# LayerXcom/zero-chain

Measured on AMD Instinct MI355X. Metric: Groth16 proofs/sec (Transfer circuit), higher is better.
Workload: dtype u32 limbs (Fq 381-bit: 14 x 28-bit; Fr 255-bit: 8 x 32-bit; modular integer arithmetic)

## Files before the change

### zero-chain_amd/csrc/msm_asm_g1.h

```cpp
#pragma once
#include "msm_accumulate.h"
#ifdef ZK_HAVE_MADD_ASM
#include "madd_asm.h"
#include "red_asm.h"

namespace zkdev {

ZK_DI void g1asm_task(uint32_t t, const Affine<Fq28>* __restrict__ table, const uint32_t* __restrict__ pairs,
                       const uint4* __restrict__ sorted, XYZZ<Fq28>* __restrict__ tsums, uint32_t* __restrict__ n_redo,
                       uint32_t* __restrict__ redo) {
    static_assert(ZK_MADD_G1_VGPRS <= 168, "the loop must fit three waves per SIMD");
    static_assert(XYZZ<Fq28>::BX >= 9 && XYZZ<Fq28>::BY >= 5, "bounds of the values handed back by the loop");
    const uint4 d = sorted[t];
    const uint32_t n = d.z;
    XYZZ<Fq28> acc = XYZZ<Fq28>::inf();
    if (n) {
        const uint32_t* pp = pairs + d.x;
        const uint32_t pr = pp[0];
        const Affine<Fq28> p = table[pr >> 1];
        if (n == 1) {
            acc = XYZZ<Fq28>{p.x, (pr & 1u) ? neg_b<Fq28::MO>(p.y) : p.y, Fq28::one(), Fq28::one()};
        } else {
            u32x16 X = fq28_vec(p.x), Y = fq28_vec(p.y), ZZ = fq28_vec(Fq28::one()), ZZZ = ZZ;
            if (pr & 1u) {
// ... 2 lines not shown
            }
            const uint64_t pa = (uint64_t)(uintptr_t)pp, ta = (uint64_t)(uintptr_t)table;
            X[14] = (uint32_t)pa;
            X[15] = (uint32_t)(pa >> 32);
            Y[14] = n;
            ZZ[14] = (uint32_t)ta;
            ZZ[15] = (uint32_t)(ta >> 32);
            asm volatile(ZK_MADD_G1_ASM
                         : "+{v[0:15]}"(X), "+{v[16:31]}"(Y), "+{v[32:47]}"(ZZ), "+{v[48:63]}"(ZZZ)
                         :
                         : ZK_MADD_G1_ASM_CLOBBERS);
            acc.x = fq28_from_signed<7, false>(X);
            acc.y = ((n - 1) & 1u) ? fq28_from_signed<3, true>(Y)
                                   : fq28_from_signed<2, false>(Y);
            acc.zz = fq28_from_signed_product(ZZ);
            acc.zzz = fq28_from_signed_product(ZZZ);
            if (acc.zz.is_zero_norm()) redo[atomicAdd(n_redo, 1u)] = t;
        }
    }
    tsums[d.y] = acc;
}
static __global__ void __launch_bounds__(128, 3)
k_msm_accumulate_g1asm(const Affine<Fq28>* __restrict__ table, const uint32_t* __restrict__ pairs,
                       const uint4* __restrict__ sorted, const uint32_t* __restrict__ total, XYZZ<Fq28>* __restrict__ tsums,
                       uint32_t* __restrict__ n_redo, uint32_t* __restrict__ redo) {
    const uint32_t t = blockIdx.x * blockDim.x + threadIdx.x;
    if (t < total[0]) g1asm_task(t, table, pairs, sorted, tsums, n_redo, redo);
}
static __global__ void __launch_bounds__(128, 3)
k_msm_accumulate_g1asm_persistent(const Affine<Fq28>* __restrict__ table, const uint32_t* __restrict__ pairs,
                                  const uint4* __restrict__ sorted, const uint32_t* __restrict__ total,
                                  XYZZ<Fq28>* __restrict__ tsums, uint32_t* __restrict__ n_redo, uint32_t* __restrict__ redo,
                                  uint32_t* __restrict__ next) {
    const uint32_t ntask = total[0], lane = threadIdx.x & 63u;
    for (;;) {
        uint32_t base = 0;
        if (lane == 0) base = atomicAdd(next, 64u);
        base = __builtin_amdgcn_readfirstlane(base);
        if (base >= ntask) break;
        if (base + lane < ntask) g1asm_task(base + lane, table, pairs, sorted, tsums, n_redo, redo);
    }
}

ZK_DI XYZZ<Fq28> red_asm_point(const u32x16& x, const u32x16& y, const u32x16& zz, const u32x16& zzz, bool is_inf, bool raw) {
    if (is_inf) return XYZZ<Fq28>::inf();
    if (raw) return XYZZ<Fq28>{fq28_unvec(x), fq28_unvec(y), fq28_unvec(zz), fq28_unvec(zzz)};
    return XYZZ<Fq28>{fq28_from_signed<7, false>(x),
                      fq28_from_signed<2, false>(y),
                      fq28_from_signed_product(zz), fq28_from_signed_product(zzz)};
}
static __global__ void __launch_bounds__(64, 2)
k_msm_reduce1_g1asm(const XYZZ<Fq28>* __restrict__ tsums, const uint32_t* __restrict__ cnt, const uint32_t* __restrict__ toff,
                    const uint32_t* __restrict__ task_base, XYZZ<Fq28>* __restrict__ S, XYZZ<Fq28>* __restrict__ A, uint32_t nb,
                    uint32_t L, uint32_t* __restrict__ n_fallback) {
    static_assert(ZK_RED_G1_VGPRS <= 256, "the loop must fit two waves per SIMD");
    static_assert(sizeof(XYZZ<Fq28>) == 224, "the loop loads 224-byte partial sums");
    const uint32_t T = nb / L;
    const uint32_t bx = (blockIdx.x + blockIdx.y) % gridDim.x;
    const uint32_t t = bx * blockDim.x + threadIdx.x;
    if (t >= T) return;
    const uint32_t job = blockIdx.y;
    const size_t b0 = (size_t)job * nb + (size_t)t * L;
    const XYZZ<Fq28>* ts = tsums + task_base[job];
    u32x16 X = {}, Y = {}, ZZ = {}, ZZZ = {}, AX, AY, AZZ, AZZZ;
    const uint64_t pc = (uint64_t)(uintptr_t)(cnt + b0), pt = (uint64_t)(uintptr_t)(toff + b0), pp = (uint64_t)(uintptr_t)ts;
    X[14] = (uint32_t)pc;
    X[15] = (uint32_t)(pc >> 32);
    Y[14] = (uint32_t)pt;
    Y[15] = (uint32_t)(pt >> 32);
    ZZ[14] = (uint32_t)pp;
    ZZ[15] = (uint32_t)(pp >> 32);
    ZZZ[14] = L;
    asm volatile(ZK_RED_G1_ASM
                 : "+{v[0:15]}"(X), "+{v[16:31]}"(Y), "+{v[32:47]}"(ZZ), "+{v[48:63]}"(ZZZ), "={v[64:79]}"(AX), "={v[80:95]}"(AY),
                   "={v[96:111]}"(AZZ), "={v[112:127]}"(AZZZ)
                 :
                 : ZK_RED_G1_ASM_CLOBBERS);
    const uint32_t flags = ZZZ[15];
    XYZZ<Fq28> run = red_asm_point(X, Y, ZZ, ZZZ, (flags & ZK_RED_FLAG_RUN_INF) != 0, (flags & ZK_RED_FLAG_RUN_RAW) != 0);
    XYZZ<Fq28> acc = red_asm_point(AX, AY, AZZ, AZZZ, (flags & ZK_RED_FLAG_ACC_INF) != 0, (flags & ZK_RED_FLAG_ACC_RAW) != 0);
    if ((!(flags & ZK_RED_FLAG_RUN_INF) && run.zz.is_zero_norm()) || (!(flags & ZK_RED_FLAG_ACC_INF) && acc.zz.is_zero_norm())) {
        atomicAdd(n_fallback, 1u);
        run = XYZZ<Fq28>::inf();
        acc = XYZZ<Fq28>::inf();
        for (int k = (int)L - 1; k >= 0; k--) {
            if (cnt[b0 + k]) run = xadd(run, ts[toff[b0 + k]]);
            if (k >= 1) acc = xadd(acc, run);
        }
    }
    S[(size_t)job * T + t] = run;
    A[(size_t)job * T + t] = acc;
}
static __global__ void __launch_bounds__(64, 2)
k_msm_reduce1_g1asm_sf(const XYZZ<Fq28>* __restrict__ tsums, const uint32_t* __restrict__ cnt, const uint32_t* __restrict__ toff,
                       const uint32_t* __restrict__ task_base, XYZZ<Fq28>* __restrict__ S, XYZZ<Fq28>* __restrict__ A, uint32_t nb,
                       uint32_t L, uint32_t* __restrict__ n_fallback, uint32_t* __restrict__ fallback) {
    const uint32_t T = nb / L;
    const uint32_t bx = (blockIdx.x + blockIdx.y) % gridDim.x;
    const uint32_t t = bx * 64u + lane_of_wave(0u);
    if (t >= T) return;
    const uint32_t job = blockIdx.y;
    size_t b0 = (size_t)job * nb + (size_t)t * L;
    const XYZZ<Fq28>* ts = tsums + task_base[job];
    u32x16 X = {}, Y = {}, ZZ = {}, ZZZ = {}, AX, AY, AZZ, AZZZ;
    const uint64_t pc = (uint64_t)(uintptr_t)(cnt + b0), pt = (uint64_t)(uintptr_t)(toff + b0), pp = (uint64_t)(uintptr_t)ts;
    X[14] = (uint32_t)pc;
    X[15] = (uint32_t)(pc >> 32);
    Y[14] = (uint32_t)pt;
    Y[15] = (uint32_t)(pt >> 32);
    ZZ[14] = (uint32_t)pp;
    ZZ[15] = (uint32_t)(pp >> 32);
    ZZZ[14] = L;
    asm volatile(ZK_RED_G1_ASM
                 : "+{v[0:15]}"(X), "+{v[16:31]}"(Y), "+{v[32:47]}"(ZZ), "+{v[48:63]}"(ZZZ), "={v[64:79]}"(AX), "={v[80:95]}"(AY),
                   "={v[96:111]}"(AZZ), "={v[112:127]}"(AZZZ)
                 :
                 : ZK_RED_G1_ASM_CLOBBERS_MIN);
    uint32_t opaque0 = 0;
    asm volatile("" : "+s"(opaque0));
    const uint32_t t2 = bx * 64u + lane_of_wave(opaque0);
    const uint32_t flags = ZZZ[15];
    XYZZ<Fq28> run = red_asm_point(X, Y, ZZ, ZZZ, (flags & ZK_RED_FLAG_RUN_INF) != 0, (flags & ZK_RED_FLAG_RUN_RAW) != 0);
    XYZZ<Fq28> acc = red_asm_point(AX, AY, AZZ, AZZZ, (flags & ZK_RED_FLAG_ACC_INF) != 0, (flags & ZK_RED_FLAG_ACC_RAW) != 0);
    if ((!(flags & ZK_RED_FLAG_RUN_INF) && run.zz.is_zero_norm()) || (!(flags & ZK_RED_FLAG_ACC_INF) && acc.zz.is_zero_norm()))
        fallback[atomicAdd(n_fallback, 1u)] = job * T + t2;
    S[(size_t)job * T + t2] = run;
    A[(size_t)job * T + t2] = acc;
}
static __global__ void __launch_bounds__(64, MsmOcc<Fq28>::red)
k_msm_reduce1_redo(const XYZZ<Fq28>* __restrict__ tsums, const uint32_t* __restrict__ cnt, const uint32_t* __restrict__ toff,
                   const uint32_t* __restrict__ task_base, XYZZ<Fq28>* __restrict__ S, XYZZ<Fq28>* __restrict__ A, uint32_t nb,
                   uint32_t L, const uint32_t* __restrict__ n_fallback, const uint32_t* __restrict__ fallback) {
    const uint32_t T = nb / L, n = n_fallback[0];
    for (uint32_t i = blockIdx.x * blockDim.x + threadIdx.x; i < n; i += gridDim.x * blockDim.x) {
        const uint32_t node = fallback[i], job = node / T, t = node % T;
        const size_t b0 = (size_t)job * nb + (size_t)t * L;
        const XYZZ<Fq28>* ts = tsums + task_base[job];
        XYZZ<Fq28> run = XYZZ<Fq28>::inf(), acc = XYZZ<Fq28>::inf();
        for (int k = (int)L - 1; k >= 0; k--) {
            if (cnt[b0 + k]) run = xadd(run, ts[toff[b0 + k]]);
            if (k >= 1) acc = xadd(acc, run);
        }
        S[node] = run;
        A[node] = acc;
    }
}

}
#endif
```

### zero-chain_amd/csrc/msm_g1.cpp

```cpp
#define ZK_MSM_GROUP_INSTANTIATE 1
#include "msm_group_impl.h"
#include "msm_sort.h"
#include "msm_asm_g1.h"

namespace zkrt {

zk_status msm_sort_pairs(const MsmPlan& p, hipStream_t st, const MsmSortBufs& w, uint32_t nb, uint32_t c, const zkdev::MsmRecode& rc,
                         const zkdev::MsmSelSet& sel_set) {
    const size_t nj = p.nj;
    const MsmJob* dj = w.jobs;
    if (p.lds_sort) {
        ProfScope ps("msm_sort_lds", st);
        ZK_LAUNCH_SYNC(zkdev::k_msm_sort_lds, dim3((unsigned)nj), dim3(zkdev::MSM_SORT_THREADS), (size_t)nb * 4, st, dj, c, w.cnt, w.off, w.toff,
                       w.ntasks, w.pairs, p.seg, hook_env("ZKAMD_DEBUG_SORT") ? (uint32_t)atoi(hook_env("ZKAMD_DEBUG_SORT")) : 0u, sel_set, rc);
        return ZK_OK;
    }
    const uint32_t fine_log = p.fine_log, fine = 1u << fine_log, n_coarse = p.n_coarse, per_wg = zkdev::MSM_COARSE_SCALARS;
    const dim3 gridc(p.coarse_wgs, (unsigned)nj);
    uint32_t* coarse_cnt = w.coarse;
    uint32_t* coarse_off = coarse_cnt + nj * (size_t)n_coarse;
    uint32_t* bin_tasks = coarse_off + nj * (size_t)n_coarse;
    uint32_t* bin_tbase = bin_tasks + nj * (size_t)n_coarse;
    HIP_TRY(hipMemsetAsync(coarse_cnt, 0, nj * (size_t)n_coarse * 4, st));
    {
        ProfScope ps("msm_sort_coarse", st);
        ZK_LAUNCH_SYNC(zkdev::k_msm_coarse_count, gridc, dim3(256), 0, st, dj, c, fine_log, n_coarse, coarse_cnt, w.blockbase, per_wg, sel_set, rc);
        ZK_LAUNCH_SYNC(zkdev::k_msm_coarse_scan, dim3((unsigned)nj), dim3(zkdev::MSM_SORT_THREADS), 0, st,
                       (const uint32_t*)coarse_cnt, coarse_off, (uint32_t*)nullptr, n_coarse);
        ZK_LAUNCH_SYNC(zkdev::k_msm_coarse_scatter, gridc, dim3(256), 0, st, dj, c, fine_log, n_coarse,
                       (const uint32_t*)coarse_off, (const uint32_t*)w.blockbase, w.rank, per_wg, sel_set, rc);
    }
    {
        ProfScope ps("msm_sort_fine", st);
        ZK_LAUNCH_SYNC(zkdev::k_msm_fine_sort, dim3(n_coarse, (unsigned)nj), dim3(zkdev::MSM_SORT_THREADS), 0, st, dj,
                       (const uint2*)w.rank, (const uint32_t*)coarse_cnt, (const uint32_t*)coarse_off, fine, nb, w.cnt, w.off, w.toff,
                       bin_tasks, w.pairs, p.seg);
        ZK_LAUNCH_SYNC(zkdev::k_msm_coarse_scan, dim3((unsigned)nj), dim3(zkdev::MSM_SORT_THREADS), 0, st,
                       (const uint32_t*)bin_tasks, bin_tbase, w.ntasks, n_coarse);
        ZK_LAUNCH(zkdev::k_msm_task_offsets, dim3((nb + 255) / 256, (unsigned)nj), dim3(256), 0, st, w.toff,
                  (const uint32_t*)bin_tbase, nb, fine_log, n_coarse);
    }
    return ZK_OK;
}

zk_status msm_order_tasks(const MsmPlan& p, hipStream_t st, const MsmSortBufs& w, uint32_t nb) {
    const uint32_t nj = (uint32_t)p.nj;
    const dim3 gridb((nb + 255) / 256, nj);
    uint32_t* lenhist = w.hist;
    uint32_t* cursor = lenhist + p.n_class;
    ProfScope ps("msm_task_sort", st);
    ZK_LAUNCH_SYNC(zkdev::k_msm_task_hist, gridb, dim3(256), 0, st, w.cnt, lenhist, nb, p.seg);
    ZK_LAUNCH_SYNC(zkdev::k_msm_task_base, dim3(1), dim3(zkdev::MSM_SORT_THREADS), 0, st, lenhist, w.tclass, w.n_tasks, nj, p.seg);
    ZK_LAUNCH_SYNC(zkdev::k_msm_task_place, gridb, dim3(256), 0, st, w.cnt, w.off, w.toff, w.tbase, w.tclass, cursor, w.sorted, w.n_heavy,
                   w.heavy, nb, nj, p.merge_inline, p.seg, w.n_light, w.light);
    return ZK_OK;
}

#ifdef ZK_HAVE_RED_ASM
template <>
void launch_red_asm<zkdev::Fq28>(const zkdev::XYZZ<zkdev::Fq28>* tsums, const uint32_t* cnt, const uint32_t* toff, const uint32_t* tbase,
                                 zkdev::XYZZ<zkdev::Fq28>* S, zkdev::XYZZ<zkdev::Fq28>* A, uint32_t nb, uint32_t L, dim3 grid,
                                 hipStream_t st, uint32_t* n_fallback, uint32_t* fallback) {
    if (kernel_form(1)) {
        ZK_LAUNCH(zkdev::k_msm_reduce1_g1asm_sf, grid, dim3(64), 0, st, tsums, cnt, toff, tbase, S, A, nb, L, n_fallback, fallback);
        ZK_LAUNCH(zkdev::k_msm_reduce1_redo, dim3(256), dim3(64), 0, st, tsums, cnt, toff, tbase, S, A, nb, L, (const uint32_t*)n_fallback,
                  (const uint32_t*)fallback);
    } else {
        ZK_LAUNCH(zkdev::k_msm_reduce1_g1asm, grid, dim3(64), 0, st, tsums, cnt, toff, tbase, S, A, nb, L, n_fallback);
    }
}
#endif
#ifdef ZK_HAVE_MADD_ASM
int persist_wgs(int group) {
    static const int v1 = getenv("ZKAMD_G1_PERSIST") ? atoi(getenv("ZKAMD_G1_PERSIST")) : 6;
    static const int v2 = getenv("ZKAMD_G2_PERSIST") ? atoi(getenv("ZKAMD_G2_PERSIST")) : 4;
    return group == 2 ? v2 : v1;
}
template <>
void launch_asm_loop<zkdev::Fq28>(const zkdev::Affine<zkdev::Fq28>* table, const uint32_t* pairs, const uint4* sorted,
                                  const uint32_t* d_total, zkdev::XYZZ<zkdev::Fq28>* tsums, uint32_t* d_nredo, uint32_t* redo,
                                  unsigned blocks, hipStream_t st) {
    if (persist_wgs() > 0 && blocks > 256u * (unsigned)persist_wgs())
        ZK_LAUNCH(zkdev::k_msm_accumulate_g1asm_persistent, dim3(256u * (unsigned)persist_wgs()), dim3(128), 0, st, table, pairs, sorted,
                  d_total, tsums, d_nredo, redo, d_nredo + 1);
    else
        ZK_LAUNCH(zkdev::k_msm_accumulate_g1asm, dim3(blocks), dim3(128), 0, st, table, pairs, sorted, d_total, tsums, d_nredo, redo);
    ZK_LAUNCH_SYNC(zkdev::k_msm_accumulate_redo<zkdev::Fq28>, dim3(1024), dim3(64), 0, st, table, pairs, sorted,
                   (const uint32_t*)d_nredo, (const uint32_t*)redo, tsums);
}
#endif

zk_status calibrate_g1_reduce(const zkdev::Affine<zkdev::Fq28>* table, uint32_t n1, float ms[2]) {
#ifdef ZK_HAVE_RED_ASM
    typedef zkdev::XYZZ<zkdev::Fq28> P1;
    const uint32_t nj = 256, nb = 4096, L = 8, T = nb / L, n_sums = 1u << 16;
    DevBuf sums, cnt, toff, tbase, S, A, ctr, list;
    ZK_TRY(sums.ensure((size_t)n_sums * sizeof(P1)));
    ZK_TRY(cnt.ensure((size_t)nj * nb * 4));
    ZK_TRY(toff.ensure((size_t)nj * nb * 4));
    ZK_TRY(tbase.ensure(nj * 4));
    ZK_TRY(S.ensure((size_t)nj * T * sizeof(P1)));
    ZK_TRY(A.ensure((size_t)nj * T * sizeof(P1)));
    ZK_TRY(ctr.ensure(4));
    ZK_TRY(list.ensure((size_t)nj * T * 4));
    HIP_TRY(hipMemsetAsync(tbase.p, 0, nj * 4, g_stream));
    ZK_LAUNCH(zkdev::k_calib_buckets<zkdev::Fq28>, dim3(nj * nb / 256), dim3(256), 0, g_stream, table, n1, sums.as<P1>(), n_sums,
              cnt.as<uint32_t>(), toff.as<uint32_t>(), nj * nb);
    const dim3 grid(T / 64, nj);
    ZK_TRY(timed_best([&] {
        (void)hipMemsetAsync(ctr.p, 0, 4, g_stream);
        ZK_LAUNCH(zkdev::k_msm_reduce1_g1asm, grid, dim3(64), 0, g_stream, (const P1*)sums.as<P1>(), (const uint32_t*)cnt.as<uint32_t>(),
                  (const uint32_t*)toff.as<uint32_t>(), (const uint32_t*)tbase.as<uint32_t>(), S.as<P1>(), A.as<P1>(), nb, L, ctr.as<uint32_t>());
    }, &ms[0]));
    ZK_TRY(timed_best([&] {
        (void)hipMemsetAsync(ctr.p, 0, 4, g_stream);
        ZK_LAUNCH(zkdev::k_msm_reduce1_g1asm_sf, grid, dim3(64), 0, g_stream, (const P1*)sums.as<P1>(), (const uint32_t*)cnt.as<uint32_t>(),
                  (const uint32_t*)toff.as<uint32_t>(), (const uint32_t*)tbase.as<uint32_t>(), S.as<P1>(), A.as<P1>(), nb, L, ctr.as<uint32_t>(),
                  list.as<uint32_t>());
        ZK_LAUNCH(zkdev::k_msm_reduce1_redo, dim3(256), dim3(64), 0, g_stream, (const P1*)sums.as<P1>(), (const uint32_t*)cnt.as<uint32_t>(),
                  (const uint32_t*)toff.as<uint32_t>(), (const uint32_t*)tbase.as<uint32_t>(), S.as<P1>(), A.as<P1>(), nb, L,
                  (const uint32_t*)ctr.as<uint32_t>(), (const uint32_t*)list.as<uint32_t>());
    }, &ms[1]));
    HIP_TRY(hipStreamSynchronize(g_stream));
#else
    (void)table; (void)n1;
    ms[0] = ms[1] = 0.f;
#endif
    return ZK_OK;
}

ZK_MSM_GROUP_DEFINE(zkhost::Fq, zkdev::Fq)

}

#ifdef ZK_TEST_HOOKS
extern "C" zk_status zk_hook_msm_plan(int is_g2, uint32_t c, const uint32_t* n, size_t n_jobs, uint32_t vb_digit, int has_asm_loop,
                                      int has_asm_reduce, uint64_t* out, size_t out_words) try {
    using namespace zkrt;
    if (!n || !n_jobs || !out || c < 2 || c > 22) return fail(ZK_ERR_INVALID_ARGUMENT, "bad argument");
    std::vector<MsmJob> jobs(n_jobs, MsmJob{});
    for (size_t k = 0; k < n_jobs; k++) {
        jobs[k].n = n[k];
        jobs[k].vb_digit = vb_digit;
    }
    MsmPlan p;
    if (msm_plan(p, is_g2 != 0, c, 1u << (c - 2), vb_digit ? 1u : zkdev::msm_max_digits(c), jobs.data(), n_jobs, has_asm_loop != 0,
                 has_asm_reduce != 0, MsmTunables::read(is_g2 != 0)) != ZK_OK)
        return fail(p.status, p.refusal);
    const MsmPlan::Bytes& b = p.bytes;
    const uint64_t f[] = {p.seg, p.few, p.coop_l1, p.coop_rb, p.merge_inline, p.heavy_cap, p.light_cap, p.use_light, p.big_launch, p.acc_asm,
                          p.red_asm, p.L, p.T, p.nbits, p.log2_2l, p.s_stride, p.nsplit, p.lds_sort, p.fine_log, p.n_coarse, p.coarse_wgs,
                          p.heavy_blocks, p.medium_max, p.max_n, p.total, p.total_tasks, p.n_buckets, p.n_class,
                          b.jobs_d, b.bucket, b.per_job, b.hist, b.heavy, b.light, b.tclass, b.sorted, b.tsums, b.pairs, b.red_r, b.red_w, b.red_t,
                          b.pin_jobs, b.rank, b.blockbase, b.coarse, b.redo, b.result, n_jobs};
    const size_t nf = sizeof(f) / sizeof(f[0]);
    if (out_words < nf + 2 * n_jobs) return fail(ZK_ERR_INVALID_ARGUMENT, "output too short");
    std::copy(f, f + nf, out);
    std::copy(p.pair_base.begin(), p.pair_base.end(), out + nf);
    std::copy(p.tbase.begin(), p.tbase.end(), out + nf + n_jobs);
    return ZK_OK;
} ZK_ABI_CATCH
#endif
```

### zero-chain_amd/csrc/msm_group.h

```cpp
#pragma once
#include <stdio.h>
#include <stdlib.h>
#include <string.h>
#include <string>
#include <vector>
#include <algorithm>
#include <utility>
#include <mutex>
#include "../../include/zkamd.h"
#include "gpu_rt.h"
#include "host_common.h"
#include "host_math.h"
#include "msm_types.h"
#include "coop_tail.h"
#include "msm_plan.h"

namespace zkrt {

inline uint32_t pick_window(size_t n, int group) {
    const char* env = getenv(group == 2 ? "ZKAMD_WINDOW_BITS_G2" : group == 3 ? "ZKAMD_WINDOW_BITS_G1A" : "ZKAMD_WINDOW_BITS_G1");
    if (!env) env = getenv("ZKAMD_WINDOW_BITS");
    if (env && atoi(env) >= 2 && atoi(env) <= 22) return (uint32_t)atoi(env);
    const char* benv = getenv(group == 2 ? "ZKAMD_BUCKET_COST_G2" : "ZKAMD_BUCKET_COST_G1");
    const double beta = benv && atof(benv) > 0 ? atof(benv) : (group == 2 ? 12.0 : group == 1 ? 4.0 : 6.0);
    uint32_t best = 2;
    double best_cost = 1e300;
    for (uint32_t c = 2; c <= 22; c++) {
        double cost = 254.0 / (c + 1) * (double)(n ? n : 1) + beta * (double)((size_t)1 << (c - 2));
        if (cost < best_cost) {
            best_cost = cost;
            best = c;
        }
    }
    return best;
}

template <class HF, class DF>
zk_status check_points_dev(const zkdev::Affine<DF>* d_pts, size_t n, const char* what);
template <class HF, class DF>
zk_status check_points_host(const std::vector<zkhost::Affine<HF>>& pts, const char* what);
template <class DF>
zk_status import_affine_dev(const void* d_src, zkdev::Affine<DF>* dst, size_t n, hipStream_t st);
template <class DF>
zk_status build_table_dev(zkdev::Affine<DF>* table, size_t n, uint32_t npos, DevBuf& scratch, uint32_t n_mult, uint32_t j0, hipStream_t st);

struct KernelForms {
    bool done = false;
    uint32_t form[2] = {0, 0};
    float ms[4] = {0, 0, 0, 0};
};
inline std::mutex g_forms_mu;
inline KernelForms g_forms[64];
inline uint32_t kernel_form(int which) {
    static const int forced = [] {
        const char* e = getenv("ZKAMD_KERNEL_FORM");
        return !e ? -1 : !strcmp(e, "free") ? 1 : !strcmp(e, "scratch") ? 0 : -1;
    }();
    if (forced >= 0) return (uint32_t)forced;
    return g_forms[g_device & 63].form[which];
}

template <class DF>
constexpr bool asm_loop() { return false; }
template <class DF>
void launch_asm_loop(const zkdev::Affine<DF>*, const uint32_t*, const uint4*, const uint32_t*, zkdev::XYZZ<DF>*, uint32_t*,
                            uint32_t*, unsigned, hipStream_t) {}
template <class DF>
constexpr bool asm_reduce() { return false; }
template <class DF>
void launch_red_asm(const zkdev::XYZZ<DF>*, const uint32_t*, const uint32_t*, const uint32_t*, zkdev::XYZZ<DF>*, zkdev::XYZZ<DF>*,
                           uint32_t, uint32_t, dim3, hipStream_t, uint32_t*, uint32_t*) {}
#ifdef ZK_HAVE_RED_ASM
template <> constexpr bool asm_reduce<zkdev::Fq28>() { return true; }
template <>
void launch_red_asm<zkdev::Fq28>(const zkdev::XYZZ<zkdev::Fq28>* tsums, const uint32_t* cnt, const uint32_t* toff, const uint32_t* tbase,
                                 zkdev::XYZZ<zkdev::Fq28>* S, zkdev::XYZZ<zkdev::Fq28>* A, uint32_t nb, uint32_t L, dim3 grid,
                                 hipStream_t st, uint32_t* n_fallback, uint32_t* fallback);
#endif
#ifdef ZK_HAVE_MADD_ASM
int persist_wgs(int group = 1);
template <> constexpr bool asm_loop<zkdev::Fq28>() { return true; }
template <> constexpr bool asm_loop<zkdev::Fq2x>() { return true; }
template <>
void launch_asm_loop<zkdev::Fq28>(const zkdev::Affine<zkdev::Fq28>* table, const uint32_t* pairs, const uint4* sorted,
                                  const uint32_t* d_total, zkdev::XYZZ<zkdev::Fq28>* tsums, uint32_t* d_nredo, uint32_t* redo,
                                  unsigned blocks, hipStream_t st);
template <>
void launch_asm_loop<zkdev::Fq2x>(const zkdev::Affine<zkdev::Fq2x>* table, const uint32_t* pairs, const uint4* sorted,
                                  const uint32_t* d_total, zkdev::XYZZ<zkdev::Fq2x>* tsums, uint32_t* d_nredo, uint32_t* redo,
                                  unsigned blocks, hipStream_t st);
#endif

struct MsmSortBufs {
    const MsmJob* jobs;
    uint32_t *cnt, *off, *toff, *ntasks, *pairs, *blockbase, *coarse;
    uint2* rank;
    uint32_t *hist, *tclass, *tbase;
    uint4* sorted;
    uint32_t *heavy, *light;
    uint32_t *n_tasks, *n_heavy, *n_light;
};
zk_status msm_sort_pairs(const MsmPlan& p, hipStream_t st, const MsmSortBufs& w, uint32_t nb, uint32_t c, const zkdev::MsmRecode& rc,
                         const zkdev::MsmSelSet& sel_set);
zk_status msm_order_tasks(const MsmPlan& p, hipStream_t st, const MsmSortBufs& w, uint32_t nb);

template <class HF, class DF>
struct MsmGroup {
    typedef zkhost::Affine<HF> HAffine;
    typedef zkhost::Point<HF> HPoint;
    typedef zkdev::Affine<DF> DAffine;
// ... 133 lines not shown
```

### zero-chain_amd/csrc/msm_group_impl.h

```cpp
#pragma once
#include "msm_group.h"
#include "msm_accumulate.h"
#include "msm_reduce.h"
#include "msm_point_kernels.h"

namespace zkrt {

template <class DF>
zk_status import_affine_dev(const void* d_src, zkdev::Affine<DF>* dst, size_t n, hipStream_t st) {
    if (!n) return ZK_OK;
    ZK_LAUNCH(zkdev::k_import_affine<DF>, dim3((unsigned)((n + 127) / 128)), dim3(128), 0, st, (const uint32_t*)d_src, dst, (uint32_t)n);
    HIP_TRY(hipGetLastError());
    return ZK_OK;
}

template <class DF>
zk_status build_table_dev(zkdev::Affine<DF>* table, size_t n, uint32_t npos, DevBuf& scratch, uint32_t n_mult, uint32_t j0, hipStream_t st) {
    ZK_TRY(scratch.ensure((size_t)zkdev::MSM_TABLE_CHUNK * 5 * sizeof(DF) * n));
    ZK_LAUNCH(zkdev::k_msm_build_table<DF>, dim3((unsigned)((n + 127) / 128)), dim3(128), 0, st, table, (uint32_t)n, npos, scratch.as<DF>(),
              n_mult, j0);
    HIP_TRY(hipGetLastError());
    return ZK_OK;
}

// ... 267 lines not shown
    ZK_LAUNCH_SYNC(zkdev::k_msm_merge_heavy<DF>,
                   dim3(lane_heavy_blocks + (light_buckets + zkdev::MSM_MERGE_THREADS - 1) / zkdev::MSM_MERGE_THREADS),
                   dim3(zkdev::MSM_MERGE_THREADS), 0, st, (const uint32_t*)heavy.as<uint32_t>(), (const uint32_t*)d_nheavy,
                   (const uint32_t*)cnt.as<uint32_t>(), (const uint32_t*)toff.as<uint32_t>(),
                   (const uint32_t*)tbase.as<uint32_t>(), tsums.as<DPoint>(), nb, seg, lane_heavy_blocks, light_buckets,
                   merge_inline, min_heavy);
    if (p.use_light)
        ZK_LAUNCH_SYNC(zkdev::k_msm_merge_light<DF>, dim3((unsigned)std::min<size_t>((p.light_cap + 63) / 64, 2048)), dim3(64), 0, st,
                       (const uint32_t*)light.as<uint32_t>(), (const uint32_t*)counter(p, N_LIGHT), (const uint32_t*)cnt.as<uint32_t>(),
                       (const uint32_t*)toff.as<uint32_t>(), (const uint32_t*)tbase.as<uint32_t>(), tsums.as<DPoint>(), nb, seg);
    return ZK_OK;
}

template <class HF, class DF>
zk_status MsmGroup<HF, DF>::level1(const MsmPlan& p, hipStream_t st) {
    const uint32_t nj = (uint32_t)p.nj, L = p.L;
    const dim3 grid((p.T + 63) / 64, nj);
    DPoint *R = node_s(), *W = node_w();
    if (p.coop_l1) {
        zkcoop::level1<DF>(tsums.as<DPoint>(), cnt.as<uint32_t>(), toff.as<uint32_t>(), tbase.as<uint32_t>(), R, W, nb, L, nj, st);
    } else if (p.red_asm) {
        launch_red_asm<DF>(tsums.as<DPoint>(), cnt.as<uint32_t>(), toff.as<uint32_t>(), tbase.as<uint32_t>(), R, W, nb, L, grid, st,
                           counter(p, N_FALLBACK), redo.as<uint32_t>());
        if (hook_env("ZKAMD_DEBUG_REDO")) dump_redo(p, st, true);
    } else {
        ZK_LAUNCH(zkdev::k_msm_suffix_buckets<DF>, grid, dim3(64), 0, st, tsums.as<DPoint>(), cnt.as<uint32_t>(),
                  toff.as<uint32_t>(), tbase.as<uint32_t>(), R, nb, L, p.few ? 0u : 1u , p.seg);
        ZK_LAUNCH(zkdev::k_msm_segsum<DF>, grid, dim3(64), 0, st, (const DPoint*)R, (const DPoint*)nullptr, W, nb, L,
                  1u, 1u, 1u);
    }
    return ZK_OK;
}

template <class HF, class DF>
zk_status MsmGroup<HF, DF>::tail(const MsmPlan& p, hipStream_t st) {
    const uint32_t nj = (uint32_t)p.nj, nbits = p.nbits;
    if (p.few) {
        DPoint* parts = red_t.as<DPoint>();
        DPoint* Y = p.nsplit > 1 ? parts + p.nj * (size_t)(nbits + 1) * p.nsplit : parts;
        zkcoop::planes<DF>(node_s(), p.s_stride, node_w(), Y, parts, p.T, nbits, nj, st);
        zkcoop::combine<DF>(Y, job_sums(p), nbits, p.log2_2l, nj, st);
    } else {
        zkcoop::upper<DF>(node_s(), p.s_stride, node_w(), job_sums(p), p.T, p.log2_2l, p.red_asm, nj, st);
    }
    return ZK_OK;
}

template <class HF, class DF>
void MsmGroup<HF, DF>::dump_redo(const MsmPlan& p, hipStream_t st, bool after_level1) {
    (void)hipStreamSynchronize(st);
    if (after_level1) {
        uint32_t v[2] = {0, 0};
        (void)hipMemcpy(v, counter(p, N_LIGHT), 8, hipMemcpyDeviceToHost);
        fprintf(stderr, "[redo] reduction G1: %u buckets with 2..%u partials merged, %u of %zu level-1 nodes recomputed\n", v[0],
                p.merge_inline, v[1], p.nj * (size_t)p.T);
        return;
    }
    uint32_t nr = 0, tot = 0;
    (void)hipMemcpy(&nr, counter(p, N_REDO), 4, hipMemcpyDeviceToHost);
    (void)hipMemcpy(&tot, counter(p, N_TASKS), 4, hipMemcpyDeviceToHost);
    fprintf(stderr, "[redo] group %s: %u of %u tasks flagged\n", IS_G2 ? "G2" : "G1", nr, tot);
    for (uint32_t q = 0; q < nr && q < 6; q++) {
        uint32_t ti = 0;
        uint4 dsc;
        (void)hipMemcpy(&ti, redo.as<uint32_t>() + q, 4, hipMemcpyDeviceToHost);
        (void)hipMemcpy(&dsc, sorted.as<uint4>() + ti, 16, hipMemcpyDeviceToHost);
        std::vector<uint32_t> pw(dsc.z);
        (void)hipMemcpy(pw.data(), pairs.as<uint32_t>() + dsc.x, dsc.z * 4, hipMemcpyDeviceToHost);
        std::sort(pw.begin(), pw.end());
        uint32_t dup = 0, opp = 0;
        for (size_t u = 1; u < pw.size(); u++) {
            dup += pw[u] == pw[u - 1];
            opp += (pw[u] ^ pw[u - 1]) == 1u;
        }
        fprintf(stderr, "[redo]   task %u: n = %u, equal pair words %u, opposite pair words %u, first %u %u %u\n", ti, dsc.z, dup, opp,
                pw.size() > 0 ? pw[0] : 0, pw.size() > 1 ? pw[1] : 0, pw.size() > 2 ? pw[2] : 0);
    }
}

template <class HF, class DF>
void MsmGroup<HF, DF>::dump_pairs(const MsmJob& job0, hipStream_t st, const char* dir) {
    static uint32_t seen = 0;
    if (job0.vb_digit || c >= 32 || (seen >> c & 1u)) return;
    seen |= 1u << c;
    (void)hipStreamSynchronize(st);
    std::vector<uint32_t> h(nb), sc((size_t)job0.n * 8);
    std::vector<int32_t> mp(job0.map ? job0.n : 0);
    (void)hipMemcpy(h.data(), cnt.p, (size_t)nb * 4, hipMemcpyDeviceToHost);
    (void)hipMemcpy(sc.data(), job0.scalars, sc.size() * 4, hipMemcpyDeviceToHost);
    if (job0.map) (void)hipMemcpy(mp.data(), job0.map, mp.size() * 4, hipMemcpyDeviceToHost);
    uint32_t pairs_job0 = 0;
    for (uint32_t x : h) pairs_job0 += x;
    const std::string path = std::string(dir) + "/pairs_" + (IS_G2 ? "g2" : "g1") + "_c" + std::to_string(c) + ".bin";
    FILE* f = fopen(path.c_str(), "wb");
    if (!f) return;
    const uint32_t head[6] = {c, n_mult, ext, job0.n, pairs_job0, job0.map ? 1u : 0u};
    fwrite(head, 4, 6, f);
    fwrite(sc.data(), 4, sc.size(), f);
    fwrite(mp.data(), 4, mp.size(), f);
    fclose(f);
}

template <class HF, class DF>
void MsmGroup<HF, DF>::dump_heavy(const MsmPlan& p, hipStream_t st) {
    (void)hipStreamSynchronize(st);
    uint32_t nh = 0;
    (void)hipMemcpy(&nh, counter(p, N_HEAVY), 4, hipMemcpyDeviceToHost);
// ... 68 lines not shown
```

### zero-chain_amd/csrc/msm_types.h

```cpp
#pragma once
#include "dev_field.h"

#if !defined(ZK_EMU) && !defined(ZK_NO_MADD_ASM)
#define ZK_HAVE_MADD_ASM 1
#define ZK_HAVE_RED_ASM 1
#endif

namespace zkdev {

struct MsmJob {
    const uint32_t* scalars;
    const int32_t* map;
    uint32_t n;
    uint32_t table_base;
    uint32_t n_table;
    uint32_t pair_base;
    uint32_t vb_digit;
    uint32_t n_digits;
};

struct MsmSelRange {
    const uint8_t* sel;
    const int32_t* alt;
    uint32_t job0, n_jobs, stride, first, n, alt_w;
// ... 6 lines not shown
    if (!job.map) return (int32_t)i;
    int32_t pos = job.map[i];
#pragma unroll
    for (int h = 0; h < 2; h++) {
        const MsmSelRange& r = S.r[h];
        const uint32_t p = j - r.job0, k = i - r.first;
        if (r.sel && p < r.n_jobs && k < r.n) {
            const uint32_t l = r.sel[(size_t)p * r.stride + k];
            if (l >= 3u) pos = l - 3u < r.alt_w ? r.alt[(size_t)k * r.alt_w + (l - 3u)] : -1;
        }
    }
    return pos;
}

template <class F> struct MsmOcc;
#ifndef ZK_OCC_G1_ACC
#define ZK_OCC_G1_ACC 2
#endif
#ifndef ZK_OCC_G1_RED
#define ZK_OCC_G1_RED 3
#endif
#ifndef ZK_OCC_G2_ACC
#define ZK_OCC_G2_ACC 2
#endif
#ifndef ZK_OCC_G2_RED
#define ZK_OCC_G2_RED 2
#endif
#ifndef ZK_OCC_G1_TAIL
#define ZK_OCC_G1_TAIL 2
#endif
#ifndef ZK_OCC_G2_TAIL
#define ZK_OCC_G2_TAIL 1
#endif
template <> struct MsmOcc<Fq> { static constexpr int acc = ZK_OCC_G1_ACC, red = ZK_OCC_G1_RED, tail = ZK_OCC_G1_TAIL; };
template <> struct MsmOcc<Fq2> { static constexpr int acc = ZK_OCC_G2_ACC, red = ZK_OCC_G2_RED, tail = ZK_OCC_G2_TAIL; };
template <> struct MsmOcc<Fq2x> { static constexpr int acc = ZK_OCC_G2_ACC, red = ZK_OCC_G2_RED, tail = ZK_OCC_G2_TAIL; };

constexpr uint32_t MSM_SEG_MAX = 256;
constexpr uint32_t MSM_NPOS = 255;

__host__ ZK_DI uint32_t msm_max_digits(uint32_t c) { return 254 / c + 2; }

constexpr uint32_t MSM_COARSE_MAX = 1024;
constexpr uint32_t MSM_FINE_MAX = 2048;
constexpr uint32_t MSM_COARSE_SCALARS = 1024;
#ifdef ZK_EMU
constexpr uint32_t MSM_SORT_THREADS = 64;
#else
constexpr uint32_t MSM_SORT_THREADS = 1024;
#endif
constexpr uint32_t MSM_MERGE_THREADS = 256;
constexpr uint32_t MSM_TABLE_CHUNK = 16;

constexpr uint32_t MSM_MULT_MAX = 8;
struct MsmRecode {
    const uint8_t* lut;
    uint32_t n_mult, ext;
};
__host__ ZK_DI uint32_t msm_mult_ext(uint32_t n_mult) { return n_mult <= 1 ? 0u : n_mult == 2 ? 2u : 3u; }
__host__ ZK_DI uint8_t msm_mult_choice(uint32_t v, uint32_t c, uint32_t n_mult, uint32_t ext) {
    const uint32_t half = 1u << (c - 1);
    for (uint32_t w = c + ext; w >= c; w--) {
        const uint32_t rho = v & ((1u << w) - 1u), other = (1u << w) - rho;
        for (uint32_t t = 0; t < 2; t++) {
            const uint32_t negative = (rho < other) == (t == 0) ? 0u : 1u, mag = negative ? other : rho;
            for (uint32_t j = 0; j < n_mult; j++) {
                const uint32_t m = 2 * j + 1;
                if (mag % m == 0 && mag / m < half) return (uint8_t)((w - c) | (negative << 3) | (j << 4));
            }
        }
    }
    return 0;
}

template <class F> struct HostWords;
template <> struct HostWords<Fq28> { static constexpr int N = 12; static constexpr bool GCD_INV = true; };
template <> struct HostWords<Fq2> { static constexpr int N = 24; static constexpr bool GCD_INV = false; };
template <> struct HostWords<Fq2x> { static constexpr int N = 24; static constexpr bool GCD_INV = true; };

}
```

### zero-chain_amd/csrc/prover_binding.h

```cpp
#pragma once
#include <atomic>
#include <chrono>
#include "prover_key.h"

namespace {

struct QueryPositions {
    std::vector<int32_t> pos_a, pos_b;
    std::vector<uint32_t> var_a, var_b;
    uint32_t n_a() const { return (uint32_t)var_a.size(); }
    uint32_t n_b() const { return (uint32_t)var_b.size(); }
};
QueryPositions query_positions(uint32_t n_in, uint32_t n_aux, const uint8_t* a_aux_d, const uint8_t* b_in_d, const uint8_t* b_aux_d) {
    const uint32_t nv = n_in + n_aux;
    QueryPositions Q;
    Q.pos_a.assign(nv, -1);
    Q.pos_b.assign(nv, -1);
    for (uint32_t i = 0; i < nv; i++) {
        if (i < n_in || a_aux_d[i - n_in]) {
            Q.pos_a[i] = (int32_t)Q.var_a.size();
            Q.var_a.push_back(i);
        }
        if (i < n_in ? b_in_d[i] : b_aux_d[i - n_in]) {
            Q.pos_b[i] = (int32_t)Q.var_b.size();
// ... 261 lines not shown
    }
    uint64_t merged = 0;
    for (const std::vector<Fr>& z : probes) merged += zkpairs::count_merges(pred, pred + nv, q, avail, (uint32_t)qy, z);
    Q.expect = (uint32_t)(merged / probes.size());
}
zk_status derived_pairs(zk_params* P, const zk_r1cs* R, const std::vector<HG1A>& set, uint32_t n_rows, PairBases& out) {
    zk_params::Binding::Pairs& X = P->bind.prs;
    X = zk_params::Binding::Pairs();
    const uint32_t n_in = R->sys.n_in, n_aux = R->sys.n_aux, nv = n_in + n_aux;
    zkpairs::Circuit kind;
    if (n_in == ZK_TRANSFER_N_INPUTS && n_aux == ZK_TRANSFER_N_AUX) kind = zkpairs::TRANSFER;
    else if (n_in == ZK_ANONYMOUS_N_INPUTS && n_aux == ZK_ANONYMOUS_N_AUX) kind = zkpairs::ANONYMOUS;
    else return ZK_OK;
    const zk_params::Key& K = P->key;
    if (P->enc_a.size() != (size_t)K.n_a * 96 || P->enc_b1.size() != (size_t)K.n_b1 * 96 || P->enc_b2.size() != (size_t)K.n_b2 * 192) return ZK_OK;
    const QueryPositions qp = query_positions(n_in, n_aux, R->sys.a_aux_density.data(), R->sys.b_input_density.data(), R->sys.b_aux_density.data());
    if (qp.n_a() != K.n_a || qp.n_b() != K.n_b1 || qp.n_b() != K.n_b2) return ZK_OK;
    std::vector<uint8_t> a_dense(nv), b_dense(nv);
    for (uint32_t i = 0; i < nv; i++) {
        a_dense[i] = qp.pos_a[i] >= 0;
        b_dense[i] = qp.pos_b[i] >= 0;
    }
    {
        const zkr1cs::System& sys = builtin_system(kind);
        if (sys.n_inputs != n_in || sys.n_aux != n_aux || sys.n_constraints != R->sys.n_con) return ZK_OK;
        std::vector<uint8_t> sa, sb;
        system_densities(sys, sa, sb);
        if (sa != a_dense || sb != b_dense) return ZK_OK;
    }
    const std::vector<std::vector<Fr>>& probes = zkpairs::circuit_probes(kind);
    if (probes.empty() || probes[0].size() != nv || set.size() != 2 * (size_t)n_rows + nv) return ZK_OK;
    const std::vector<int32_t> chains = zkpairs::chains_of(probes, n_in, a_dense, b_dense);
    std::vector<int32_t> pos_l(nv, -1);
    for (uint32_t i = n_in; i < nv; i++)
        if (!set[2 * (size_t)n_rows + i].is_inf()) pos_l[i] = (int32_t)(2 * n_rows + i);
    std::vector<HG1A> pts_a, pts_b1;
    const bool decoded = decode_query(P->enc_a, zkhost::g1_from_uncompressed, pts_a) && decode_query(P->enc_b1, zkhost::g1_from_uncompressed, pts_b1) &&
                         decode_query(P->enc_b2, zkhost::g2_from_uncompressed, out.b2);
    if (!decoded) return fail(ZK_ERR_IO, "internal: a query of the key does not decode a second time");
    X.links.assign(11 * (size_t)nv, -1);
    std::copy(chains.begin(), chains.end(), X.links.begin());
    std::fill(X.links.begin() + 10 * (size_t)nv, X.links.end(), 0);
    query_pairs(X, QA, chains, probes, qp.pos_a, pts_a, out.g1);
    query_pairs(X, QB2, chains, probes, qp.pos_b, out.b2, out.g2);
    query_pairs(X, QL, chains, probes, pos_l, set, out.g1);
    query_pairs(X, QB1, chains, probes, qp.pos_b, pts_b1, out.g1);
    X.ready = X.counts().any();
    return ZK_OK;
}

#ifndef ZK_TABLE_MULTIPLES_DEFAULT
#define ZK_TABLE_MULTIPLES_DEFAULT 8
#endif
uint32_t table_multiples() {
    const char* env = getenv("ZKAMD_TABLE_MULTIPLES");
    const int v = env ? atoi(env) : 0;
    return v == 1 || v == 2 || v == 4 || v == 8 ? (uint32_t)v : ZK_TABLE_MULTIPLES_DEFAULT;
}
size_t table_multiples_min() {
    const char* env = getenv("ZKAMD_TABLE_MULTIPLES_MIN");
    return env && atol(env) > 0 ? (size_t)atol(env) : 129;
}

zk_status add_table_multiples(zk_params* P) {
    zk_params::Binding& B = P->bind;
    const uint32_t asked = table_multiples();
    if (B.drv.multiples_tried || !B.g1d.table.owned) return ZK_OK;
    B.drv.multiples_tried = true;
    if (asked <= 1) return ZK_OK;
    ZK_TRY(use_device(P->key.device));
    const auto t0 = std::chrono::steady_clock::now();
    zk_status st = hook_env("ZKAMD_INJECT_TABLE_OOM") ? fail(ZK_ERR_OUT_OF_MEMORY, "injected: the table with its multiples does not fit")
                                                     : B.g1d.add_multiples(asked);
    if (st == ZK_OK && B.prs.ready) st = B.g2p.add_multiples(asked);
    if (st != ZK_OK && st != ZK_ERR_OUT_OF_MEMORY) return st;
    B.g1d_lone.alias(B.g1d, B.g1d_lone.c);
    if (B.prs.ready) {
        B.g1da.alias(B.g1d, B.g1da.c);
        B.g2p_lone.alias(B.g2p, B.g2p_lone.c);
    }
    if (getenv("ZKAMD_TRACE_HOST"))
        fprintf(stderr, "[zkamd] table multiples: %u asked%s, G1 table %u per slice %.2f GB, G2 table %u per slice %.2f GB, %.1f ms\n", asked,
                st == ZK_OK ? "" : " (out of memory)", B.g1d.n_mult, (double)B.g1d.bytes / 1e9, B.g2p.n_mult, (double)B.g2p.bytes / 1e9,
                std::chrono::duration<double, std::milli>(std::chrono::steady_clock::now() - t0).count());
    return ZK_OK;
}

zk_status ensure_derived(zk_params* P, zk_r1cs* R, bool batch) {
    if (P->bind.drv.ready && P->bind.drv.circuit == R->sys.id) return batch ? add_table_multiples(P) : ZK_OK;
    P->bind.drv.multiples_tried = false;
    const uint32_t n_in = R->sys.n_in, n_aux = R->sys.n_aux, nv = n_in + n_aux, n_con = R->sys.n_con, n_rows = n_con + n_in, k = P->key.log_m;
    const size_t m = P->key.m;
    if (!P->tab.g1.table.owned || R->sys.h_row_ptr[2].size() != (size_t)n_con + 1 || n_in != P->key.n_ic || n_aux != P->key.n_l ||
        (size_t)n_con + n_in > m || P->key.n_h + 1 != m)
        return ZK_OK;
    ZK_TRY(use_device(P->key.device));
    const auto t0 = std::chrono::steady_clock::now();
    typedef zkdev::XYZZ<zkdev::Fq> DP;
    typedef zkdev::Affine<zkdev::Fq> DA;
    P->bind.drv.ready = false;
    const DA* key = P->tab.g1.table.as<DA>();
    const std::vector<uint32_t>& rp = R->sys.h_row_ptr[2];
    const std::vector<uint32_t>& cl = R->sys.h_col[2];
    const uint32_t nnz = rp[n_con];
    std::vector<uint32_t> ptr(nv + 1, 0), t_row(nnz ? nnz : 1), each(n_rows + 1);
    std::vector<Fr> t_s(nnz ? nnz : 1);
    for (uint32_t e = 0; e < nnz; e++) ptr[cl[e] + 1]++;
    for (uint32_t i = 0; i < nv; i++) ptr[i + 1] += ptr[i];
    {
        std::vector<uint32_t> at(ptr.begin(), ptr.end() - 1);
        for (uint32_t row = 0; row < n_con; row++)
            for (uint32_t e = rp[row]; e < rp[row + 1]; e++) {
                const uint32_t slot = at[cl[e]]++;
                t_row[slot] = row;
                t_s[slot] = R->sys.h_coeff[2][e].from_mont();
            }
    }
    for (uint32_t i = 0; i <= n_rows; i++) each[i] = i;
    std::vector<int32_t> idx(m + nv);
    for (size_t pos = 0; pos < m; pos++) {
        const uint32_t e = k ? (__builtin_bitreverse32((uint32_t)pos) >> (32 - k)) : 0;
        idx[pos] = e < P->key.n_h ? (int32_t)(P->key.off_h + e) : -1;
    }
    for (uint32_t i = 0; i < nv; i++) idx[m + i] = i < n_in ? -1 : (int32_t)(P->key.off_l + (i - n_in));
    const size_t rows = std::max<size_t>(m, nnz), n_set = 2 * (size_t)n_rows + nv;
    DevBuf d_idx, d_ptr, d_each, d_row, d_s, d_tw, d_w, d_sl, d_sm, d_se, src, ping, pong, lam, mk, terms, tbl, all, stage;
    for (DevBuf* b : {&d_idx, &d_ptr, &d_each, &d_row, &d_s, &d_tw, &d_w, &d_sl, &d_sm, &d_se, &src, &ping, &pong, &lam, &mk, &terms, &tbl, &all, &stage})
        b->is_public = true;
    const Fr ninv2 = P->tab.ntt.n_inv * P->tab.ntt.n_inv;
    const Fr wv[5] = {P->tab.ntt.w_inv, Fr::one(), ninv2, -ninv2, fr_from_u64((uint64_t)m) * P->tab.ntt.z_inv};
    ZK_TRY(d_idx.upload(idx));
    ZK_TRY(d_ptr.upload(ptr));
    ZK_TRY(d_each.upload(each));
    ZK_TRY(d_row.upload(t_row));
    ZK_TRY(d_s.upload(t_s));
    ZK_TRY(d_w.upload(wv, 5));
// ... 119 lines not shown
```

Measured before the change: 5169.

## Defer reduce1 fallback to a parallel tree-reduce redo kernel; allow 16 table multiples

```diff
diff --git a/zero-chain_amd/csrc/msm_asm_g1.h b/zero-chain_amd/csrc/msm_asm_g1.h
--- a/zero-chain_amd/csrc/msm_asm_g1.h
+++ b/zero-chain_amd/csrc/msm_asm_g1.h
@@ -78,7 +78,7 @@
 static __global__ void __launch_bounds__(64, 2)
 k_msm_reduce1_g1asm(const XYZZ<Fq28>* __restrict__ tsums, const uint32_t* __restrict__ cnt, const uint32_t* __restrict__ toff,
                     const uint32_t* __restrict__ task_base, XYZZ<Fq28>* __restrict__ S, XYZZ<Fq28>* __restrict__ A, uint32_t nb,
-                    uint32_t L, uint32_t* __restrict__ n_fallback) {
+                    uint32_t L, uint32_t* __restrict__ n_fallback, uint32_t* __restrict__ fallback) {
     static_assert(ZK_RED_G1_VGPRS <= 256, "the loop must fit two waves per SIMD");
     static_assert(sizeof(XYZZ<Fq28>) == 224, "the loop loads 224-byte partial sums");
     const uint32_t T = nb / L;
@@ -105,15 +105,8 @@
     const uint32_t flags = ZZZ[15];
     XYZZ<Fq28> run = red_asm_point(X, Y, ZZ, ZZZ, (flags & ZK_RED_FLAG_RUN_INF) != 0, (flags & ZK_RED_FLAG_RUN_RAW) != 0);
     XYZZ<Fq28> acc = red_asm_point(AX, AY, AZZ, AZZZ, (flags & ZK_RED_FLAG_ACC_INF) != 0, (flags & ZK_RED_FLAG_ACC_RAW) != 0);
-    if ((!(flags & ZK_RED_FLAG_RUN_INF) && run.zz.is_zero_norm()) || (!(flags & ZK_RED_FLAG_ACC_INF) && acc.zz.is_zero_norm())) {
-        atomicAdd(n_fallback, 1u);
-        run = XYZZ<Fq28>::inf();
-        acc = XYZZ<Fq28>::inf();
-        for (int k = (int)L - 1; k >= 0; k--) {
-            if (cnt[b0 + k]) run = xadd(run, ts[toff[b0 + k]]);
-            if (k >= 1) acc = xadd(acc, run);
-        }
-    }
+    if ((!(flags & ZK_RED_FLAG_RUN_INF) && run.zz.is_zero_norm()) || (!(flags & ZK_RED_FLAG_ACC_INF) && acc.zz.is_zero_norm()))
+        fallback[atomicAdd(n_fallback, 1u)] = job * T + t;
     S[(size_t)job * T + t] = run;
     A[(size_t)job * T + t] = acc;
 }
@@ -153,22 +146,35 @@
     S[(size_t)job * T + t2] = run;
     A[(size_t)job * T + t2] = acc;
 }
+constexpr uint32_t MSM_RED1_FAN_MAX = 32;
 static __global__ void __launch_bounds__(64, MsmOcc<Fq28>::red)
 k_msm_reduce1_redo(const XYZZ<Fq28>* __restrict__ tsums, const uint32_t* __restrict__ cnt, const uint32_t* __restrict__ toff,
                    const uint32_t* __restrict__ task_base, XYZZ<Fq28>* __restrict__ S, XYZZ<Fq28>* __restrict__ A, uint32_t nb,
                    uint32_t L, const uint32_t* __restrict__ n_fallback, const uint32_t* __restrict__ fallback) {
-    const uint32_t T = nb / L, n = n_fallback[0];
-    for (uint32_t i = blockIdx.x * blockDim.x + threadIdx.x; i < n; i += gridDim.x * blockDim.x) {
+    ZK_SHARED XYZZ<Fq28> sm[MSM_RED1_FAN_MAX];
+    const uint32_t T = nb / L, n = n_fallback[0], k = threadIdx.x;
+    if (L > MSM_RED1_FAN_MAX) return;
+    for (uint32_t i = blockIdx.x; i < n; i += gridDim.x) {
         const uint32_t node = fallback[i], job = node / T, t = node % T;
         const size_t b0 = (size_t)job * nb + (size_t)t * L;
         const XYZZ<Fq28>* ts = tsums + task_base[job];
-        XYZZ<Fq28> run = XYZZ<Fq28>::inf(), acc = XYZZ<Fq28>::inf();
-        for (int k = (int)L - 1; k >= 0; k--) {
-            if (cnt[b0 + k]) run = xadd(run, ts[toff[b0 + k]]);
-            if (k >= 1) acc = xadd(acc, run);
+        XYZZ<Fq28> run = XYZZ<Fq28>::inf();
+        if (k < L && cnt[b0 + k]) run = ts[toff[b0 + k]];
+        for (uint32_t d = 1; d < L; d <<= 1) {
+            if (k < L) sm[k] = run;
+            __syncthreads();
+            if (k + d < L) run = xadd(run, sm[k + d]);
+            __syncthreads();
         }
-        S[node] = run;
-        A[node] = acc;
+        if (k == 0) S[node] = run;
+        XYZZ<Fq28> acc = k >= 1 && k < L ? run : XYZZ<Fq28>::inf();
+        for (uint32_t d = L >> 1; d >= 1; d >>= 1) {
+            if (k < 2 * d) sm[k] = acc;
+            __syncthreads();
+            if (k < d) acc = xadd(acc, sm[k + d]);
+            __syncthreads();
+        }
+        if (k == 0) A[node] = acc;
     }
 }
 
diff --git a/zero-chain_amd/csrc/msm_g1.cpp b/zero-chain_amd/csrc/msm_g1.cpp
--- a/zero-chain_amd/csrc/msm_g1.cpp
+++ b/zero-chain_amd/csrc/msm_g1.cpp
@@ -61,13 +61,12 @@
 void launch_red_asm<zkdev::Fq28>(const zkdev::XYZZ<zkdev::Fq28>* tsums, const uint32_t* cnt, const uint32_t* toff, const uint32_t* tbase,
                                  zkdev::XYZZ<zkdev::Fq28>* S, zkdev::XYZZ<zkdev::Fq28>* A, uint32_t nb, uint32_t L, dim3 grid,
                                  hipStream_t st, uint32_t* n_fallback, uint32_t* fallback) {
-    if (kernel_form(1)) {
+    if (kernel_form(1))
         ZK_LAUNCH(zkdev::k_msm_reduce1_g1asm_sf, grid, dim3(64), 0, st, tsums, cnt, toff, tbase, S, A, nb, L, n_fallback, fallback);
-        ZK_LAUNCH(zkdev::k_msm_reduce1_redo, dim3(256), dim3(64), 0, st, tsums, cnt, toff, tbase, S, A, nb, L, (const uint32_t*)n_fallback,
-                  (const uint32_t*)fallback);
-    } else {
-        ZK_LAUNCH(zkdev::k_msm_reduce1_g1asm, grid, dim3(64), 0, st, tsums, cnt, toff, tbase, S, A, nb, L, n_fallback);
-    }
+    else
+        ZK_LAUNCH(zkdev::k_msm_reduce1_g1asm, grid, dim3(64), 0, st, tsums, cnt, toff, tbase, S, A, nb, L, n_fallback, fallback);
+    ZK_LAUNCH(zkdev::k_msm_reduce1_redo, dim3(1024), dim3(64), 0, st, tsums, cnt, toff, tbase, S, A, nb, L, (const uint32_t*)n_fallback,
+              (const uint32_t*)fallback);
 }
 #endif
 #ifdef ZK_HAVE_MADD_ASM
@@ -107,19 +106,24 @@
     ZK_LAUNCH(zkdev::k_calib_buckets<zkdev::Fq28>, dim3(nj * nb / 256), dim3(256), 0, g_stream, table, n1, sums.as<P1>(), n_sums,
               cnt.as<uint32_t>(), toff.as<uint32_t>(), nj * nb);
     const dim3 grid(T / 64, nj);
+    auto redo = [&] {
+        ZK_LAUNCH(zkdev::k_msm_reduce1_redo, dim3(1024), dim3(64), 0, g_stream, (const P1*)sums.as<P1>(), (const uint32_t*)cnt.as<uint32_t>(),
+                  (const uint32_t*)toff.as<uint32_t>(), (const uint32_t*)tbase.as<uint32_t>(), S.as<P1>(), A.as<P1>(), nb, L,
+                  (const uint32_t*)ctr.as<uint32_t>(), (const uint32_t*)list.as<uint32_t>());
+    };
     ZK_TRY(timed_best([&] {
         (void)hipMemsetAsync(ctr.p, 0, 4, g_stream);
         ZK_LAUNCH(zkdev::k_msm_reduce1_g1asm, grid, dim3(64), 0, g_stream, (const P1*)sums.as<P1>(), (const uint32_t*)cnt.as<uint32_t>(),
-                  (const uint32_t*)toff.as<uint32_t>(), (const uint32_t*)tbase.as<uint32_t>(), S.as<P1>(), A.as<P1>(), nb, L, ctr.as<uint32_t>());
+                  (const uint32_t*)toff.as<uint32_t>(), (const uint32_t*)tbase.as<uint32_t>(), S.as<P1>(), A.as<P1>(), nb, L, ctr.as<uint32_t>(),
+                  list.as<uint32_t>());
+        redo();
     }, &ms[0]));
     ZK_TRY(timed_best([&] {
         (void)hipMemsetAsync(ctr.p, 0, 4, g_stream);
         ZK_LAUNCH(zkdev::k_msm_reduce1_g1asm_sf, grid, dim3(64), 0, g_stream, (const P1*)sums.as<P1>(), (const uint32_t*)cnt.as<uint32_t>(),
                   (const uint32_t*)toff.as<uint32_t>(), (const uint32_t*)tbase.as<uint32_t>(), S.as<P1>(), A.as<P1>(), nb, L, ctr.as<uint32_t>(),
                   list.as<uint32_t>());
-        ZK_LAUNCH(zkdev::k_msm_reduce1_redo, dim3(256), dim3(64), 0, g_stream, (const P1*)sums.as<P1>(), (const uint32_t*)cnt.as<uint32_t>(),
-                  (const uint32_t*)toff.as<uint32_t>(), (const uint32_t*)tbase.as<uint32_t>(), S.as<P1>(), A.as<P1>(), nb, L,
-                  (const uint32_t*)ctr.as<uint32_t>(), (const uint32_t*)list.as<uint32_t>());
+        redo();
     }, &ms[1]));
     HIP_TRY(hipStreamSynchronize(g_stream));
 #else
diff --git a/zero-chain_amd/csrc/msm_group.h b/zero-chain_amd/csrc/msm_group.h
--- a/zero-chain_amd/csrc/msm_group.h
+++ b/zero-chain_amd/csrc/msm_group.h
@@ -51,11 +51,16 @@
 };
 inline std::mutex g_forms_mu;
 inline KernelForms g_forms[64];
+inline int kernel_form_forced() {
+    const char* e = getenv("ZKAMD_KERNEL_FORM");
+    return !e ? -1 : !strcmp(e, "free") ? 1 : !strcmp(e, "scratch") ? 0 : -1;
+}
 inline uint32_t kernel_form(int which) {
-    static const int forced = [] {
-        const char* e = getenv("ZKAMD_KERNEL_FORM");
-        return !e ? -1 : !strcmp(e, "free") ? 1 : !strcmp(e, "scratch") ? 0 : -1;
-    }();
+#ifdef ZK_TEST_HOOKS
+    const int forced = kernel_form_forced();
+#else
+    static const int forced = kernel_form_forced();
+#endif
     if (forced >= 0) return (uint32_t)forced;
     return g_forms[g_device & 63].form[which];
 }
diff --git a/zero-chain_amd/csrc/msm_group_impl.h b/zero-chain_amd/csrc/msm_group_impl.h
--- a/zero-chain_amd/csrc/msm_group_impl.h
+++ b/zero-chain_amd/csrc/msm_group_impl.h
@@ -343,7 +343,7 @@
     if (after_level1) {
         uint32_t v[2] = {0, 0};
         (void)hipMemcpy(v, counter(p, N_LIGHT), 8, hipMemcpyDeviceToHost);
-        fprintf(stderr, "[redo] reduction G1: %u buckets with 2..%u partials merged, %u of %zu level-1 nodes recomputed\n", v[0],
+        fprintf(stderr, "[redo] reduction G1: %u buckets with 2..%u partials merged, %u of %zu level-1 nodes listed and recomputed\n", v[0],
                 p.merge_inline, v[1], p.nj * (size_t)p.T);
         return;
     }
diff --git a/zero-chain_amd/csrc/msm_types.h b/zero-chain_amd/csrc/msm_types.h
--- a/zero-chain_amd/csrc/msm_types.h
+++ b/zero-chain_amd/csrc/msm_types.h
@@ -82,12 +82,12 @@
 constexpr uint32_t MSM_MERGE_THREADS = 256;
 constexpr uint32_t MSM_TABLE_CHUNK = 16;
 
-constexpr uint32_t MSM_MULT_MAX = 8;
+constexpr uint32_t MSM_MULT_MAX = 16;
 struct MsmRecode {
     const uint8_t* lut;
     uint32_t n_mult, ext;
 };
-__host__ ZK_DI uint32_t msm_mult_ext(uint32_t n_mult) { return n_mult <= 1 ? 0u : n_mult == 2 ? 2u : 3u; }
+__host__ ZK_DI uint32_t msm_mult_ext(uint32_t n_mult) { return n_mult <= 1 ? 0u : n_mult == 2 ? 2u : n_mult <= 8 ? 3u : 4u; }
 __host__ ZK_DI uint8_t msm_mult_choice(uint32_t v, uint32_t c, uint32_t n_mult, uint32_t ext) {
     const uint32_t half = 1u << (c - 1);
     for (uint32_t w = c + ext; w >= c; w--) {
diff --git a/zero-chain_amd/csrc/prover_binding.h b/zero-chain_amd/csrc/prover_binding.h
--- a/zero-chain_amd/csrc/prover_binding.h
+++ b/zero-chain_amd/csrc/prover_binding.h
@@ -337,11 +337,13 @@
 #ifndef ZK_TABLE_MULTIPLES_DEFAULT
 #define ZK_TABLE_MULTIPLES_DEFAULT 8
 #endif
-uint32_t table_multiples() {
-    const char* env = getenv("ZKAMD_TABLE_MULTIPLES");
+inline uint32_t table_multiples_of(const char* name, uint32_t otherwise) {
+    const char* env = getenv(name);
     const int v = env ? atoi(env) : 0;
-    return v == 1 || v == 2 || v == 4 || v == 8 ? (uint32_t)v : ZK_TABLE_MULTIPLES_DEFAULT;
-}
+    return v == 1 || v == 2 || v == 4 || v == 8 || v == 16 ? (uint32_t)v : otherwise;
+}
+uint32_t table_multiples() { return table_multiples_of("ZKAMD_TABLE_MULTIPLES", ZK_TABLE_MULTIPLES_DEFAULT); }
+uint32_t table_multiples_g2() { return table_multiples_of("ZKAMD_TABLE_MULTIPLES_G2", table_multiples()); }
 size_t table_multiples_min() {
     const char* env = getenv("ZKAMD_TABLE_MULTIPLES_MIN");
     return env && atol(env) > 0 ? (size_t)atol(env) : 129;
@@ -349,24 +351,33 @@
 
 zk_status add_table_multiples(zk_params* P) {
     zk_params::Binding& B = P->bind;
-    const uint32_t asked = table_multiples();
+    const uint32_t asked = table_multiples(), asked_g2 = table_multiples_g2();
     if (B.drv.multiples_tried || !B.g1d.table.owned) return ZK_OK;
     B.drv.multiples_tried = true;
-    if (asked <= 1) return ZK_OK;
+    if (asked <= 1 && asked_g2 <= 1) return ZK_OK;
     ZK_TRY(use_device(P->key.device));
     const auto t0 = std::chrono::steady_clock::now();
-    zk_status st = hook_env("ZKAMD_INJECT_TABLE_OOM") ? fail(ZK_ERR_OUT_OF_MEMORY, "injected: the table with its multiples does not fit")
-                                                     : B.g1d.add_multiples(asked);
-    if (st == ZK_OK && B.prs.ready) st = B.g2p.add_multiples(asked);
-    if (st != ZK_OK && st != ZK_ERR_OUT_OF_MEMORY) return st;
+    bool short_of_memory = false;
+    auto grow = [&](auto& group, uint32_t want) -> zk_status {
+        if (want <= 1) return ZK_OK;
+        zk_status st = hook_env("ZKAMD_INJECT_TABLE_OOM") ? fail(ZK_ERR_OUT_OF_MEMORY, "injected: the table with its multiples does not fit")
+                                                         : group.add_multiples(want);
+        if (st == ZK_ERR_OUT_OF_MEMORY) {
+            short_of_memory = true;
+            st = want > 8 ? group.add_multiples(8) : ZK_OK;
+        }
+        return st == ZK_ERR_OUT_OF_MEMORY ? ZK_OK : st;
+    };
+    ZK_TRY(grow(B.g1d, asked));
+    if (B.prs.ready) ZK_TRY(grow(B.g2p, asked_g2));
     B.g1d_lone.alias(B.g1d, B.g1d_lone.c);
     if (B.prs.ready) {
         B.g1da.alias(B.g1d, B.g1da.c);
         B.g2p_lone.alias(B.g2p, B.g2p_lone.c);
     }
     if (getenv("ZKAMD_TRACE_HOST"))
-        fprintf(stderr, "[zkamd] table multiples: %u asked%s, G1 table %u per slice %.2f GB, G2 table %u per slice %.2f GB, %.1f ms\n", asked,
-                st == ZK_OK ? "" : " (out of memory)", B.g1d.n_mult, (double)B.g1d.bytes / 1e9, B.g2p.n_mult, (double)B.g2p.bytes / 1e9,
+        fprintf(stderr, "[zkamd] table multiples: %u asked, %u for G2%s, G1 table %u per slice %.2f GB, G2 table %u per slice %.2f GB, %.1f ms\n", asked,
+                asked_g2, short_of_memory ? " (out of memory)" : "", B.g1d.n_mult, (double)B.g1d.bytes / 1e9, B.g2p.n_mult, (double)B.g2p.bytes / 1e9,
                 std::chrono::duration<double, std::milli>(std::chrono::steady_clock::now() - t0).count());
     return ZK_OK;
 }
```

Measured after the change: 5170, median of 2. About the same (+0.0%).
